# jspenmar/slowtv_monodepth

Measured on AMD Instinct MI355X. Metric: training images/sec (640×192, 3-frame) at 1/2/4/8 MI355X; warp+SSIM HBM GB/s, higher is better.
Workload: dtype f32

## Files before the change

### slowtv_monodepth_amd/conv_routing.py

```python
from __future__ import annotations

import torch

from ._lib import Unsupported

_MODE = 'auto'
_ROUTES: dict = {}
_AB_WARMUPS, _AB_ROUNDS, _AB_MARGIN = 2, 5, 0.97
_DECLINED = (Unsupported, ValueError)


def set_conv_route(mode: str = 'auto'):
    global _MODE
    if mode not in ('auto', 'mfma', 'miopen'): raise ValueError(mode)
    _MODE = mode
    _ROUTES.clear()


def conv_routes() -> dict:
    return dict(_ROUTES)


_COARSE_W_MAX, _COARSE_C_MIN = 80, 256
_Z_FWD_WGT = [dict(px_min=1000, ch_max=511), dict(px_min=2400)]
STATIC_RULES = {
    'padded': {'fwd': [dict(thin=True), dict(thin=False, px_min=20000, c_co_max=128*64), dict(thin=False, coarse=True, px_min=1000)],
               'data': [dict(thin=True), dict(thin=False, px_min=5000, c_max=256), dict(thin=False, coarse=True, px_min=1000)],
               'wgt': [dict(thin=False, px_min=20000, co_max=64), dict(thin=False, coarse=True, px_min=2400)]},
    'bf16': {'fwd': [dict(thin=True)], 'data': [dict(thin=True)], 'wgt': [dict(thin=True)]},
    'zpad': {'fwd': _Z_FWD_WGT, 'data': [dict(px_min=1000)], 'wgt': _Z_FWD_WGT},
    'stem': {'fwd': [dict(px_min=20000)], 'wgt': [dict(px_min=20000)]},
}
_FAMILY_OF_SUFFIX = {'': 'padded', 'bf16': 'bf16', 'z': 'zpad', 's': 'stem'}
_BOUNDS = {'px_min': lambda v, B, C, CO, h, w: B*h*w >= v,
           'c_max': lambda v, B, C, CO, h, w: C <= v,
           'co_max': lambda v, B, C, CO, h, w: CO <= v,
           'c_co_max': lambda v, B, C, CO, h, w: C*CO <= v,
           'ch_max': lambda v, B, C, CO, h, w: max(C, CO) <= v,
           'thin': lambda v, B, C, CO, h, w: (CO == 16) == v,
           'coarse': lambda v, B, C, CO, h, w: (w <= _COARSE_W_MAX and C >= _COARSE_C_MIN) == v}


STRIDED_RULES = {
    's2': {'fwd': [dict(px_min=5000)], 'wgt': []},
}


TRANSPOSED_RULES = {
    't2': {'data': [dict(px_min=5000)]},
}


def static_rule(op, B, C, CO, h, w) -> bool:
    kind, _, suffix = op.partition('_')
    if suffix in _FAMILY_OF_SUFFIX: clauses = STATIC_RULES[_FAMILY_OF_SUFFIX[suffix]][kind]
    elif suffix in STRIDED_RULES or suffix not in TRANSPOSED_RULES: clauses = STRIDED_RULES[suffix][kind]
    else: clauses = TRANSPOSED_RULES[suffix][kind]
    return any(all(_BOUNDS[name](v, B, C, CO, h, w) for name, v in clause.items()) for clause in clauses)


def may_serve(key, unknown=True) -> bool:
    if _MODE != 'auto': return _MODE == 'mfma'
    r = _ROUTES.get(key)
    if r is None: return static_rule(*key) if torch.cuda.is_initialized() and _capturing() else unknown
    return r[0]


_capturing = torch.cuda.is_current_stream_capturing


def _time_interleaved(run_mfma, run_ref, rounds):
    ev = [[torch.cuda.Event(enable_timing=True) for _ in range(3)] for _ in range(rounds)]
    for e in ev:
        e[0].record(); run_mfma(); e[1].record(); run_ref(); e[2].record()
    torch.cuda.synchronize()
    return [e[0].elapsed_time(e[1])*1e3 for e in ev], [e[1].elapsed_time(e[2])*1e3 for e in ev]


def _conv_route(op, B, C, CO, h, w, run_mfma, run_ref) -> bool:
    if _MODE != 'auto': return _MODE == 'mfma'
    key = (op, B, C, CO, h, w)
    r = _ROUTES.get(key)
    if r is None:
        if _capturing(): return static_rule(op, B, C, CO, h, w)
        for _ in range(_AB_WARMUPS): run_mfma(); run_ref()
        us_m, us_r = _time_interleaved(run_mfma, run_ref, _AB_ROUNDS)
        t_m, t_r = sorted(us_m)[_AB_ROUNDS//2], sorted(us_r)[_AB_ROUNDS//2]
        r = _ROUTES[key] = (t_m < _AB_MARGIN*t_r, t_m, t_r)
    return r[0]


def serve(key, run_mfma, run_ref, *, eligible, force=False):
    if not eligible: return run_ref()
    if force: return run_mfma()
    try:
        use = _conv_route(*key, run_mfma, run_ref)
    except _DECLINED:
        _ROUTES[key] = (False, float('nan'), float('nan'))
        use = False
    if use:
        try:
            return run_mfma()
        except _DECLINED:
            pass
    return run_ref()
```

### slowtv_monodepth_amd/csrc/smd_conv_s2.hip

```cpp
#include "smd_common.h"
#include "smd_kernels.h"
#include "smd_conv_mfma_dev.h"
#include <algorithm>
#include <type_traits>

namespace smd {

namespace {

constexpr int kS2Pix = 388;

template <int P>
__global__ __launch_bounds__(256, 2) void k_conv_s2_fwd(const float* __restrict__ x, const uint4* __restrict__ wp, float* __restrict__ out,
                                                        int CK, int M, int H, int W, int ho, int wo, int TR, int TCW, int KS, int kc_per_split,
                                                        size_t split_stride, unsigned gx, unsigned gy, unsigned gz) {
  constexpr int NPIX = kS2Pix, kBuf = P*NPIX*2;
  __shared__ uint4 tile[2*kBuf];
  const int lane = threadIdx.x & 63, wall = __builtin_amdgcn_readfirstlane(threadIdx.x >> 6), j = lane & 31, g = lane >> 5;
  const int MT = M >> 5, MG = (MT + 3) >> 2;
  const unsigned nblk = (unsigned)(MG*KS)*gx*gy*gz, lid = xcd_block_id(nblk);
  if (lid >= nblk) return;
  const int mg_own = (int)(lid % MG)*4 + wall, mg = min(mg_own, MT - 1), ks = (lid/MG) % KS;
  const unsigned tl = lid/(MG*KS);
  const int x0 = (int)(tl % gx)*TCW, y0 = (int)((tl/gx) % gy)*TR, b = (int)(tl/(gx*gy));
  const int PW = 2*TCW + 1, PWH = TCW + 1, NP = (2*TR + 1)*PW;
  const int KC = CK >> 4, kc0 = ks*kc_per_split, kc1 = min(KC, kc0 + kc_per_split);
  const size_t plane = (size_t)H*W;
  const float* src = x + (size_t)b*CK*plane;

  int lbase[2];
  bool have[2];
#pragma unroll
  for (int nt = 0; nt < 2; ++nt) {
    const int p = nt*32 + j, r = p/TCW, c = p - r*TCW;
    have[nt] = p < TR*TCW && y0 + r < ho && x0 + c < wo;
    lbase[nt] = have[nt] ? 2*r*PW + c : 0;
  }

  using Stage = PatchStager<256, NPIX, P, float, true>;
  constexpr int TRIPS = Stage::TRIPS;
  Stage stage;
#pragma unroll
  for (int t = 0; t < TRIPS; ++t) {
    const int item = Stage::item(t), half = item >= NPIX ? 1 : 0, pix = item - half*NPIX;
    const int rp = pix/PW, q = pix - rp*PW, col = q < PWH ? 2*q : 2*(q - PWH) + 1;
    const int yy = 2*y0 + rp - 1, xx = 2*x0 + col - 1;
    stage.pofs[t] = (pix < NP && yy >= 0 && yy < H && xx >= 0 && xx < W) ? yy*W + xx : -1;
  }
  float v[TRIPS][8];
  auto request = [&](int kc) { stage.request(src, plane, kc, v); };
  auto file_trip = [&](int buf, int t) { stage.file_trip(tile, buf, t, v); };

  f32x16 acc[2], lo[2];
#pragma unroll
  for (int nt = 0; nt < 2; ++nt)
#pragma unroll
    for (int r = 0; r < 16; ++r) { acc[nt][r] = 0.f; lo[nt][r] = 0.f; }

  bf16x8 A[5][P], Bf[2][2][P];
  const uint4* wq = wp + ((size_t)mg*KC*9*P)*64 + lane;
  auto fetch_a = [&](bf16x8 (&dst)[P], int kc, int tap) {
#pragma unroll
    for (int p = 0; p < P; ++p) dst[p] = as_frag(wq[(size_t)((kc*9 + tap)*P + p)*64]);
  };
  auto read_b = [&](bf16x8 (&dst)[2][P], int buf, int tap) {
    const int ky = tap/3, kx = tap % 3;
    const int d = ky*PW + (kx & 1)*PWH + (kx >> 1);
#pragma unroll
    for (int nt = 0; nt < 2; ++nt) Stage::read(tile, buf, lbase[nt] + d, g, dst[nt]);
  };
  auto chunk = [&](int kc, int cur, auto more_tag) {
    constexpr bool MORE = decltype(more_tag)::value;
    read_b(Bf[0], cur, 0);
#pragma unroll
    for (int tap = 0; tap < 9; ++tap) {
      if (tap < 8) read_b(Bf[(tap + 1) & 1], cur, tap + 1);
      split_mfma<P>(A[tap % 5], Bf[tap & 1], acc, lo);
      if (tap <= 4) fetch_a(A[(tap + 4) % 5], kc, tap + 4);
      else if (MORE && tap >= 6) fetch_a(A[tap - 6], kc + 1, tap - 6);
      if (MORE && tap == 8) fetch_a(A[3], kc + 1, 3);
      if (MORE && tap == 4) request(kc + 1);
      if (MORE && tap >= 6) {
#pragma unroll
        for (int t = 0; t < TRIPS; ++t) if (t*3/TRIPS == tap - 6) file_trip(cur ^ 1, t);
      }
      __builtin_amdgcn_sched_barrier(0);
    }
    __syncthreads();
  };

  if (kc0 < kc1) {
    request(kc0);
#pragma unroll
    for (int tap = 0; tap < 4; ++tap) fetch_a(A[tap], kc0, tap);
    stage.file(tile, 0, v);
  }
  __syncthreads();
  int kc = kc0;
  for (; kc + 1 < kc1; ++kc) chunk(kc, (kc - kc0) & 1, std::true_type{});
  if (kc < kc1) chunk(kc, (kc - kc0) & 1, std::false_type{});

  if (mg_own >= MT) return;
  float* dst = out + (size_t)ks*split_stride;
#pragma unroll
  for (int nt = 0; nt < 2; ++nt) {
    if (!have[nt]) continue;
    const int p = nt*32 + j, r = p/TCW, c = p - r*TCW;
#pragma unroll
    for (int rr = 0; rr < 16; ++rr) {
      const int m = mg*32 + mfma32_row(rr, g);
      dst[(((size_t)b*M + m)*ho + y0 + r)*wo + x0 + c] = acc[nt][rr] + lo[nt][rr];
    }
  }
}

__global__ __launch_bounds__(256) void k_s2_split_sum(const float* __restrict__ part, float* __restrict__ out, size_t n4, int KS) {
  const size_t i = (size_t)blockIdx.x*256 + threadIdx.x;
  if (i >= n4) return;
  const f4* p = reinterpret_cast<const f4*>(part);
  f4 s = p[i];
  for (int k = 1; k < KS; ++k) s += p[(size_t)k*n4 + i];
  reinterpret_cast<f4*>(out)[i] = s;
}

void s2_tile(int ho, int wo, int& TR, int& TCW) {
  double best = -1.0; int best_patch = 0;
  TR = 1; TCW = 1;
  for (int tcw = std::min(wo, 64); tcw >= 1; --tcw) {
    int tr = std::min(64/tcw, ho);
    while (tr > 1 && (2*tr + 1)*(2*tcw + 1) > kS2Pix) --tr;
    const int patch = (2*tr + 1)*(2*tcw + 1);
    const double useful = (double)ho*wo/((double)ceil_div(ho, tr)*ceil_div(wo, tcw)*64.0);
    if (useful > best + 1e-9 || (useful > best - 1e-9 && patch < best_patch)) { best = useful; best_patch = patch; TR = tr; TCW = tcw; }
  }
}
struct S2Shape { int TR, TCW, KS, kcs; unsigned gx, gy, gz; dim3 grid; size_t out_elems; };
S2Shape s2_fwd_shape(int B, int C, int CO, int ho, int wo) {
  S2Shape s;
  s2_tile(ho, wo, s.TR, s.TCW);
  s.gx = ceil_div(wo, s.TCW); s.gy = ceil_div(ho, s.TR); s.gz = B;
  const int KC = C >> 4, MG = ceil_div(CO >> 5, 4);
  const long long base = (long long)s.gx*s.gy*s.gz*MG;
  int ks = 1;
  if (base < 384) ks = (int)std::min<long long>(std::max(KC/2, 1), (512 + base - 1)/base);
  s.kcs = ceil_div(KC, ks); s.KS = ceil_div(KC, s.kcs);
  s.grid = dim3(8*(unsigned)ceil_div(base*s.KS, 8ll));
  s.out_elems = (size_t)B*CO*ho*wo;
  return s;
}

struct S2W {
  static constexpr int CB = 64, COB = 64, STRIP = 32, P = 3;
  static constexpr int XO = 20, XCH = 36;
  static constexpr int GCH = 20;
  static constexpr int XROW = CB*XCH, XPIECE = 3*XROW, GPIECE = COB*GCH;
  static constexpr int XITEMS = CB*2*17, XTR = (XITEMS + 255)/256;
  static constexpr int GTR = COB*8/256;
};

__global__ __launch_bounds__(256, 1) void k_conv_s2_wgrad(const float* __restrict__ x, const float* __restrict__ gy, float* __restrict__ partial,
                                                          int B, int C, int CO, int H, int W, int ho, int wo, int rows_per_block, int spb) {
  using T = S2W;
  constexpr int P = T::P, XO = T::XO, XCH = T::XCH, GCH = T::GCH, XROW = T::XROW, XPIECE = T::XPIECE, GPIECE = T::GPIECE, XTR = T::XTR, GTR = T::GTR;
  __shared__ __attribute__((aligned(16))) unsigned xs[P*XPIECE];
  __shared__ __attribute__((aligned(16))) unsigned gs[P*GPIECE];
  const int lane = threadIdx.x & 63, wv = __builtin_amdgcn_readfirstlane(threadIdx.x >> 6), j = lane & 31, g = lane >> 5;
  const int ct = wv & 1, cot = wv >> 1;
  const int CG = ceil_div(C, T::CB), COG = ceil_div(CO, T::COB);
  const int cg = blockIdx.z % CG, cog = (blockIdx.z/CG) % COG, sg = blockIdx.z/(CG*COG);
  const int x0 = blockIdx.x*T::STRIP, ybeg = blockIdx.y*rows_per_block, nrows = min(rows_per_block, ho - ybeg);
  const int b0 = sg*spb, nb = min(spb, B - b0);
  const size_t xplane = (size_t)H*W, gplane = (size_t)ho*wo;

  float xv[XTR][4], gv[GTR][4];
  auto load_x = [&](const float* xb, int ir0) {
#pragma unroll
    for (int t = 0; t < XTR; ++t) {
      const int item = t*256 + (int)threadIdx.x;
      const int d = item % 17, rr = (item/17) & 1, ch = item/34, c = cg*T::CB + ch;
      const int ir = ir0 + rr, gc = 2*x0 - 1 + 4*d;
      const bool ok = item < T::XITEMS && c < C && ir >= 0 && ir < H;
      const float* rowp = xb + ((size_t)min(c, C - 1)*H + max(min(ir, H - 1), 0))*W;
#pragma unroll
      for (int k = 0; k < 4; ++k) xv[t][k] = (ok && gc + k >= 0 && gc + k < W) ? rowp[gc + k] : 0.f;
    }
  };
  auto file_x = [&](int ir0, bool both) {
#pragma unroll
    for (int t = 0; t < XTR; ++t) {
      const int item = t*256 + (int)threadIdx.x;
      const int d = item % 17, rr = (item/17) & 1, ch = item/34;
      if (item < T::XITEMS && (both || rr == 1)) {
        const int slot = (ir0 + rr + 4) % 3;
        unsigned pe[P], po[P];
        split_pair<P>(xv[t][0], xv[t][2], pe);
        split_pair<P>(xv[t][1], xv[t][3], po);
#pragma unroll
        for (int p = 0; p < P; ++p) {
          unsigned* row = xs + p*XPIECE + slot*XROW + ch*XCH;
          row[d] = pe[p];
          if (d < 16) row[XO + d] = po[p];
        }
      }
    }
  };
  auto load_g = [&](const float* gb, int yy) {
#pragma unroll
    for (int t = 0; t < GTR; ++t) {
      const int item = t*256 + (int)threadIdx.x;
      const int chn = item >> 3, co = cog*T::COB + chn, xa = x0 + 4*(item & 7);
      const float* rowp = gb + ((size_t)min(co, CO - 1)*ho + yy)*wo;
#pragma unroll
      for (int k = 0; k < 4; ++k) gv[t][k] = (co < CO && xa + k < wo) ? rowp[xa + k] : 0.f;
    }
  };
  auto file_g = [&]() {
#pragma unroll
    for (int t = 0; t < GTR; ++t) {
      const int item = t*256 + (int)threadIdx.x;
      const int chn = item >> 3, q = item & 7;
      unsigned p0[P], p1[P];
      split_pair<P>(gv[t][0], gv[t][1], p0);
      split_pair<P>(gv[t][2], gv[t][3], p1);
#pragma unroll
      for (int p = 0; p < P; ++p) {
        gs[p*GPIECE + chn*GCH + 2*q] = p0[p];
        gs[p*GPIECE + chn*GCH + 2*q + 1] = p1[p];
      }
    }
  };

  f32x16 acc[9];
#pragma unroll
  for (int t = 0; t < 9; ++t)
#pragma unroll
    for (int r = 0; r < 16; ++r) acc[t][r] = 0.f;

  for (int s = 0; s < nb; ++s) {
    const float* xb = x + (size_t)(b0 + s)*C*xplane;
    const float* gb = gy + (size_t)(b0 + s)*CO*gplane;
    load_x(xb, 2*ybeg - 2); file_x(2*ybeg - 2, false);
    load_x(xb, 2*ybeg); file_x(2*ybeg, true);
    load_g(gb, ybeg); file_g();
    __syncthreads();
    for (int r = 0; r < nrows; ++r) {
      const int yy = ybeg + r;
      const bool more = r + 1 < nrows;
      if (more) { load_x(xb, 2*yy + 2); load_g(gb, yy + 1); }
#pragma unroll
      for (int ks = 0; ks < 2; ++ks) {
        const int kd = ks*8 + g*4;
        bf16x8 A[P];
#pragma unroll
        for (int p = 0; p < P; ++p) A[p] = as_frag(*reinterpret_cast<const uint4*>(&gs[p*GPIECE + (cot*32 + j)*GCH + kd]));
#pragma unroll
        for (int ky = 0; ky < 3; ++ky) {
          const int slot = (2*yy + ky) % 3;
          bf16x8 Bx[3][P];
#pragma unroll
          for (int p = 0; p < P; ++p) {
            const unsigned* row = xs + p*XPIECE + slot*XROW + (ct*32 + j)*XCH;
            const uint4 e = *reinterpret_cast<const uint4*>(row + kd);
            const unsigned e4 = row[kd + 4];
            Bx[0][p] = as_frag(e);
            Bx[1][p] = as_frag(*reinterpret_cast<const uint4*>(row + XO + kd));
            Bx[2][p] = as_frag(uint4{__builtin_amdgcn_alignbit(e.y, e.x, 16), __builtin_amdgcn_alignbit(e.z, e.y, 16),
                                     __builtin_amdgcn_alignbit(e.w, e.z, 16), __builtin_amdgcn_alignbit(e4, e.w, 16)});
          }
          split_mfma_sum<P>(A, Bx, &acc[ky*3]);
        }
      }
      __syncthreads();
      if (more) { file_x(2*yy + 2, true); file_g(); }
      __syncthreads();
    }
  }

  const size_t blk = ((size_t)sg*gridDim.y + blockIdx.y)*gridDim.x + blockIdx.x;
  const int c = cg*T::CB + ct*32 + j;
  if (c < C) {
#pragma unroll
    for (int t = 0; t < 9; ++t)
#pragma unroll
      for (int r = 0; r < 16; ++r) {
        const int co = cog*T::COB + cot*32 + mfma32_row(r, g);
        if (co < CO) partial[((blk*9 + t)*CO + co)*C + c] = acc[t][r];
      }
  }
}

void s2_wgrad_shape(int B, int C, int CO, int ho, int wo, dim3& grid, int& rows, int& spb) {
  const int cgs = ceil_div(C, S2W::CB)*ceil_div(CO, S2W::COB), strips = ceil_div(wo, S2W::STRIP);
  const long long base = (long long)strips*B*cgs;
  const int groups = (int)std::max(1ll, std::min<long long>(256/std::max(base, 1ll), ceil_div(ho, 6)));
  rows = ceil_div(ho, groups);
  spb = 1;
  if (rows == ho && base > 512) spb = (int)std::min<long long>(B, base/256);
  grid = dim3(strips, ceil_div(ho, rows), ceil_div(B, spb)*cgs);
}
unsigned s2_wgrad_sets(int B, int C, int CO, int ho, int wo) {
  dim3 grid; int rows, spb;
  s2_wgrad_shape(B, C, CO, ho, wo, grid, rows, spb);
  return grid.x*grid.y*(unsigned)ceil_div(B, spb);
}

constexpr int kS2DPix = 128;

__device__ __forceinline__ constexpr int s2d_slot(int s) { return (int)((0x867250134ull >> (4*s)) & 15); }

template <int P>
__device__ __forceinline__ void split_mfma_two(const bf16x8 (&A0)[P], const bf16x8 (&B0)[P], f32x16& acc0, f32x16& lo0,
                                               const bf16x8 (&A1)[P], const bf16x8 (&B1)[P], f32x16& acc1, f32x16& lo1) {
  constexpr int NPROD = n_products(P);
#pragma unroll
  for (int t = 0; t < NPROD; ++t) {
    if (t == NPROD - 1) { acc0 = mfma_bf16(A0[0], B0[0], acc0); acc1 = mfma_bf16(A1[0], B1[0], acc1); }
    else {
      lo0 = mfma_bf16(A0[prod_a(P, t)], B0[prod_b(P, t)], lo0);
      lo1 = mfma_bf16(A1[prod_a(P, t)], B1[prod_b(P, t)], lo1);
    }
  }
}

template <int P>
__global__ __launch_bounds__(256, 2) void k_conv_s2_bwd_data(const float* __restrict__ gy, const uint4* __restrict__ wp, float* __restrict__ out,
                                                             int CK, int M, int H, int W, int ho, int wo, int TR, int TCW, int KS, int kc_per_split,
                                                             size_t split_stride, unsigned gx, unsigned gyb, unsigned gz) {
  constexpr int NPIX = kS2DPix, kBuf = P*NPIX*2;
  __shared__ uint4 tile[2*kBuf];
  const int lane = threadIdx.x & 63, wall = __builtin_amdgcn_readfirstlane(threadIdx.x >> 6), j = lane & 31, g = lane >> 5;
  const int MT = (M + 31) >> 5, MG = (MT + 1) >> 1;
  const unsigned nblk = (unsigned)(MG*KS)*gx*gyb*gz, lid = xcd_block_id(nblk);
  if (lid >= nblk) return;
  const int nf = wall & 1;
  const int mt_own = (int)(lid % MG)*2 + (wall >> 1), mt = min(mt_own, MT - 1), ks = (lid/MG) % KS;
  const unsigned tl = lid/(MG*KS);
  const int c0 = (int)(tl % gx)*TCW, r0 = (int)((tl/gx) % gyb)*TR, b = (int)(tl/(gx*gyb));
  const int PW = TCW + 1, NP = (TR + 1)*PW;
  const int KC = CK >> 4, kc0 = ks*kc_per_split, kc1 = min(KC, kc0 + kc_per_split);
  const size_t plane = (size_t)ho*wo;
  const float* src = gy + (size_t)b*CK*plane;

  const int p = nf*32 + j, r = p/TCW, c = p - r*TCW;
  const bool have = p < TR*TCW && r0 + r < ho && c0 + c < wo;
  const int lbase = have ? r*PW + c : 0;

  using Stage = PatchStager<256, NPIX, P, float, true>;
  constexpr int TRIPS = Stage::TRIPS;
  Stage stage;
#pragma unroll
  for (int t = 0; t < TRIPS; ++t) {
    const int item = Stage::item(t), half = item >= NPIX ? 1 : 0, pix = item - half*NPIX;
    const int rp = pix/PW, q = pix - rp*PW;
    const int yy = r0 + rp, xx = c0 + q;
    stage.pofs[t] = (pix < NP && yy < ho && xx < wo) ? yy*wo + xx : -1;
  }
  float v[TRIPS][8];
  auto request = [&](int kc) { stage.request(src, plane, kc, v); };

  f32x16 acc[4], lo[4];
#pragma unroll
  for (int q = 0; q < 4; ++q)
#pragma unroll
    for (int rr = 0; rr < 16; ++rr) { acc[q][rr] = 0.f; lo[q][rr] = 0.f; }

  bf16x8 A[5][P], Bf[2][P];
  const uint4* wq = wp + ((size_t)mt*KC*9*P)*64 + lane;
  auto fetch_a = [&](bf16x8 (&dst)[P], int kc, int s) {
#pragma unroll
    for (int pc = 0; pc < P; ++pc) dst[pc] = as_frag(wq[(size_t)((kc*9 + s2d_slot(s))*P + pc)*64]);
  };
  auto read_b = [&](bf16x8 (&dst)[P], int buf, int d) { Stage::read(tile, buf, lbase + d, g, dst); };
  auto chunk = [&](int kc, int cur, auto more_tag) {
    constexpr bool MORE = decltype(more_tag)::value;
    read_b(Bf[0], cur, 0);
    read_b(Bf[1], cur, 1);
    split_mfma_two<P>(A[0], Bf[0], acc[0], lo[0], A[1], Bf[0], acc[1], lo[1]);
    fetch_a(A[4], kc, 4); fetch_a(A[0], kc, 5);
    __builtin_amdgcn_sched_barrier(0);
    split_mfma_two<P>(A[2], Bf[0], acc[2], lo[2], A[3], Bf[0], acc[3], lo[3]);
    fetch_a(A[1], kc, 6); fetch_a(A[2], kc, 7);
    read_b(Bf[0], cur, PW);
    if (MORE) request(kc + 1);
    __builtin_amdgcn_sched_barrier(0);
    split_mfma_two<P>(A[4], Bf[1], acc[1], lo[1], A[0], Bf[1], acc[3], lo[3]);
    fetch_a(A[3], kc, 8);
    if (MORE) fetch_a(A[0], kc + 1, 0);
    read_b(Bf[1], cur, PW + 1);
    __builtin_amdgcn_sched_barrier(0);
    split_mfma_two<P>(A[1], Bf[0], acc[2], lo[2], A[2], Bf[0], acc[3], lo[3]);
    if (MORE) { fetch_a(A[1], kc + 1, 1); fetch_a(A[2], kc + 1, 2); }
    __builtin_amdgcn_sched_barrier(0);
    split_mfma<P>(A[3], Bf[1], acc[3], lo[3]);
    if (MORE) {
      fetch_a(A[3], kc + 1, 3);
      stage.file(tile, cur ^ 1, v);
    }
    __builtin_amdgcn_sched_barrier(0);
    __syncthreads();
  };

  if (kc0 < kc1) {
    request(kc0);
#pragma unroll
    for (int s = 0; s < 4; ++s) fetch_a(A[s], kc0, s);
    stage.file(tile, 0, v);
  }
  __syncthreads();
  int kc = kc0;
  for (; kc + 1 < kc1; ++kc) chunk(kc, (kc - kc0) & 1, std::true_type{});
  if (kc < kc1) chunk(kc, (kc - kc0) & 1, std::false_type{});

  if (mt_own >= MT || !have) return;
  float* dst = out + (size_t)ks*split_stride;
  const int y = 2*(r0 + r), x = 2*(c0 + c);
  const bool row1 = y + 1 < H, col1 = x + 1 < W;
  const bool pairs = (W & 1) == 0 && (reinterpret_cast<uintptr_t>(dst) & 7) == 0;
#pragma unroll
  for (int rr = 0; rr < 16; ++rr) {
    const int m = mt*32 + mfma32_row(rr, g);
    if (m >= M) continue;
    float* q = dst + (((size_t)b*M + m)*H + y)*W + x;
    const float v00 = acc[0][rr] + lo[0][rr], v01 = acc[1][rr] + lo[1][rr], v10 = acc[2][rr] + lo[2][rr], v11 = acc[3][rr] + lo[3][rr];
    if (pairs) {
      *reinterpret_cast<f32x2v*>(q) = f32x2v{v00, v01};
      if (row1) *reinterpret_cast<f32x2v*>(q + W) = f32x2v{v10, v11};
    } else {
      q[0] = v00;
      if (col1) q[1] = v01;
      if (row1) { q[W] = v10; if (col1) q[W + 1] = v11; }
    }
  }
}

void s2d_tile(int ho, int wo, int& TR, int& TCW) {
  double best = -1.0; int best_patch = 0;
  TR = 1; TCW = 1;
  for (int tcw = std::min(wo, 63); tcw >= 1; --tcw) {
    int tr = std::min(64/tcw, ho);
    while (tr > 1 && (tr + 1)*(tcw + 1) > kS2DPix) --tr;
    const int patch = (tr + 1)*(tcw + 1);
    const double useful = (double)ho*wo/((double)ceil_div(ho, tr)*ceil_div(wo, tcw)*64.0);
    if (useful > best + 1e-9 || (useful > best - 1e-9 && patch < best_patch)) { best = useful; best_patch = patch; TR = tr; TCW = tcw; }
  }
}
S2Shape s2d_shape(int B, int C, int CO, int H, int W) {
  const int ho = (H - 1)/2 + 1, wo = (W - 1)/2 + 1;
  S2Shape s;
  s2d_tile(ho, wo, s.TR, s.TCW);
  s.gx = ceil_div(wo, s.TCW); s.gy = ceil_div(ho, s.TR); s.gz = B;
  const int KC = CO >> 4, MG = ceil_div(ceil_div(C, 32), 2);
  const long long base = (long long)s.gx*s.gy*s.gz*MG;
  int ks = 1;
  if (base < 256) ks = (int)std::min<long long>(std::max(KC/2, 1), (512 + base - 1)/base);
  s.kcs = ceil_div(KC, ks); s.KS = ceil_div(KC, s.kcs);
  s.grid = dim3(8*(unsigned)ceil_div(base*s.KS, 8ll));
  s.out_elems = (size_t)B*C*H*W;
  return s;
}

}

bool conv_s2_served(int C, int CO) { return C >= 16 && C % 16 == 0 && CO >= 32 && CO % 32 == 0; }
size_t conv_s2_workspace_floats(int B, int C, int CO, int H, int W) {
  const int ho = (H - 1)/2 + 1, wo = (W - 1)/2 + 1;
  const S2Shape s = s2_fwd_shape(B, C, CO, ho, wo);
  return std::max({(size_t)64, s.KS > 1 ? (size_t)s.KS*s.out_elems : (size_t)0, partial_sets_floats(s2_wgrad_sets(B, C, CO, ho, wo), (size_t)9*CO*C)});
}
hipError_t launch_conv_s2_fwd(const float* x, const void* wp_fwd, float* y, float* split_ws, int B, int C, int CO, int H, int W, hipStream_t st) {
  const int ho = (H - 1)/2 + 1, wo = (W - 1)/2 + 1;
  const S2Shape s = s2_fwd_shape(B, C, CO, ho, wo);
  hipLaunchKernelGGL(k_conv_s2_fwd<3>, s.grid, dim3(256), 0, st, x, (const uint4*)wp_fwd, s.KS > 1 ? split_ws : y, C, CO, H, W, ho, wo, s.TR, s.TCW, s.KS, s.kcs,
                     s.out_elems, s.gx, s.gy, s.gz);
  if (s.KS > 1) {
    const size_t n4 = s.out_elems/4;
    hipLaunchKernelGGL(k_s2_split_sum, dim3((unsigned)((n4 + 255)/256)), dim3(256), 0, st, split_ws, y, n4, s.KS);
  }
  return hipGetLastError();
}
hipError_t launch_conv_s2_bwd_wgt(const float* x, const float* gy, float* g_w, float* partial, int B, int C, int CO, int H, int W, hipStream_t st) {
  const int ho = (H - 1)/2 + 1, wo = (W - 1)/2 + 1;
  dim3 grid; int rows, spb;
  s2_wgrad_shape(B, C, CO, ho, wo, grid, rows, spb);
  hipLaunchKernelGGL(k_conv_s2_wgrad, grid, dim3(256), 0, st, x, gy, partial, B, C, CO, H, W, ho, wo, rows, spb);
  return launch_partial_sets_finalize(partial, grid.x*grid.y*(unsigned)ceil_div(B, spb), 9*CO*C, SetIndexMap{CO, C}, g_w, st);
}

long long conv_s2d_blocks(int B, int C, int CO, int H, int W) { return (long long)s2d_shape(B, C, CO, H, W).grid.x; }
size_t conv_s2d_workspace_floats(int B, int C, int CO, int H, int W) {
  const S2Shape s = s2d_shape(B, C, CO, H, W);
  return std::max((size_t)64, s.KS > 1 ? (size_t)s.KS*s.out_elems : (size_t)0);
}
hipError_t launch_conv_s2_bwd_data(const float* gy, const void* wp_bwd, float* g_x, float* split_ws, int B, int C, int CO, int H, int W, hipStream_t st) {
  const int ho = (H - 1)/2 + 1, wo = (W - 1)/2 + 1;
  const S2Shape s = s2d_shape(B, C, CO, H, W);
  hipLaunchKernelGGL(k_conv_s2_bwd_data<3>, s.grid, dim3(256), 0, st, gy, (const uint4*)wp_bwd, s.KS > 1 ? split_ws : g_x, CO, C, H, W, ho, wo, s.TR, s.TCW, s.KS,
                     s.kcs, s.out_elems, s.gx, s.gy, s.gz);
  if (s.KS > 1) {
    const size_t n4 = s.out_elems/4;
    hipLaunchKernelGGL(k_s2_split_sum, dim3((unsigned)((n4 + 255)/256)), dim3(256), 0, st, split_ws, g_x, n4, s.KS);
  }
  return hipGetLastError();
}

}
```

Measured before the change: 959.3.

## Rewrite stride-2 conv weight-grad kernel with async LDS DMA ring and enable routing

Replaces the register-staged load/split/store pipeline of the stride-2 weight-gradient kernel with direct buffer-to-LDS DMA into a four-slot ring. Loads are issued ahead and waited on with vmcnt. The bf16 split now happens at fragment-build time, and each input row is reused across two output rows via alternating accumulator sets. Tile shape changes to 32 input by 128 output channels on a 16-wide strip with two blocks per CU. The grid shape is now picked by a small cost model. The static routing rule is also enabled for small-C shapes during graph capture. The aim is to hide global-load latency and cut register pressure, at the cost of tricky wait-count logic and reduced channel reuse per block.

```diff
diff --git a/slowtv_monodepth_amd/conv_routing.py b/slowtv_monodepth_amd/conv_routing.py
--- a/slowtv_monodepth_amd/conv_routing.py
+++ b/slowtv_monodepth_amd/conv_routing.py
@@ -42,7 +42,7 @@
 
 
 STRIDED_RULES = {
-    's2': {'fwd': [dict(px_min=5000)], 'wgt': []},
+    's2': {'fwd': [dict(px_min=5000)], 'wgt': [dict(c_max=64, px_min=5000)]},
 }
 
 
diff --git a/slowtv_monodepth_amd/csrc/smd_conv_s2.hip b/slowtv_monodepth_amd/csrc/smd_conv_s2.hip
--- a/slowtv_monodepth_amd/csrc/smd_conv_s2.hip
+++ b/slowtv_monodepth_amd/csrc/smd_conv_s2.hip
@@ -150,84 +150,60 @@
 }
 
 struct S2W {
-  static constexpr int CB = 64, COB = 64, STRIP = 32, P = 3;
-  static constexpr int XO = 20, XCH = 36;
-  static constexpr int GCH = 20;
-  static constexpr int XROW = CB*XCH, XPIECE = 3*XROW, GPIECE = COB*GCH;
-  static constexpr int XITEMS = CB*2*17, XTR = (XITEMS + 255)/256;
-  static constexpr int GTR = COB*8/256;
+  static constexpr int CB = 32, COB = 128, STRIP = 16, P = 3, NW = 4, D = 4;
+  static constexpr int XCS = 36, GCS = 20, XDW = CB*XCS, GDW = COB*GCS, SLOT = 2*XDW + GDW;
+  static constexpr int NX = 16*XCS/64, NG = 16*GCS/64, NDMA = NX + 2*NG;
+  static_assert(NX*64 == 16*XCS && NG*64 == 16*GCS && 2*XDW == NW*NX*64 && GDW == NW*2*NG*64, "a wave: sixteen channels of one input row, 32 of dL/dy");
+  static_assert((D - 2)*NDMA < 64 && D == 4, "the waits below are immediates of six bits, for a ring of four");
 };
 
-__global__ __launch_bounds__(256, 1) void k_conv_s2_wgrad(const float* __restrict__ x, const float* __restrict__ gy, float* __restrict__ partial,
+__global__ __launch_bounds__(256, 2) void k_conv_s2_wgrad(const float* __restrict__ x, const float* __restrict__ gy, float* __restrict__ partial,
                                                           int B, int C, int CO, int H, int W, int ho, int wo, int rows_per_block, int spb) {
   using T = S2W;
-  constexpr int P = T::P, XO = T::XO, XCH = T::XCH, GCH = T::GCH, XROW = T::XROW, XPIECE = T::XPIECE, GPIECE = T::GPIECE, XTR = T::XTR, GTR = T::GTR;
-  __shared__ __attribute__((aligned(16))) unsigned xs[P*XPIECE];
-  __shared__ __attribute__((aligned(16))) unsigned gs[P*GPIECE];
+  constexpr int P = T::P, D = T::D, XCS = T::XCS, GCS = T::GCS, XDW = T::XDW, SLOT = T::SLOT, NX = T::NX, NG = T::NG, NDMA = T::NDMA;
+  __shared__ __attribute__((aligned(16))) unsigned lds[D*SLOT];
   const int lane = threadIdx.x & 63, wv = __builtin_amdgcn_readfirstlane(threadIdx.x >> 6), j = lane & 31, g = lane >> 5;
-  const int ct = wv & 1, cot = wv >> 1;
+  const int cot = wv;
   const int CG = ceil_div(C, T::CB), COG = ceil_div(CO, T::COB);
   const int cg = blockIdx.z % CG, cog = (blockIdx.z/CG) % COG, sg = blockIdx.z/(CG*COG);
   const int x0 = blockIdx.x*T::STRIP, ybeg = blockIdx.y*rows_per_block, nrows = min(rows_per_block, ho - ybeg);
-  const int b0 = sg*spb, nb = min(spb, B - b0);
+  const int b0 = sg*spb, nsteps = nrows + 1, nsteps_all = min(spb, B - b0)*nsteps;
   const size_t xplane = (size_t)H*W, gplane = (size_t)ho*wo;
-
-  float xv[XTR][4], gv[GTR][4];
-  auto load_x = [&](const float* xb, int ir0) {
-#pragma unroll
-    for (int t = 0; t < XTR; ++t) {
-      const int item = t*256 + (int)threadIdx.x;
-      const int d = item % 17, rr = (item/17) & 1, ch = item/34, c = cg*T::CB + ch;
-      const int ir = ir0 + rr, gc = 2*x0 - 1 + 4*d;
-      const bool ok = item < T::XITEMS && c < C && ir >= 0 && ir < H;
-      const float* rowp = xb + ((size_t)min(c, C - 1)*H + max(min(ir, H - 1), 0))*W;
-#pragma unroll
-      for (int k = 0; k < 4; ++k) xv[t][k] = (ok && gc + k >= 0 && gc + k < W) ? rowp[gc + k] : 0.f;
-    }
-  };
-  auto file_x = [&](int ir0, bool both) {
-#pragma unroll
-    for (int t = 0; t < XTR; ++t) {
-      const int item = t*256 + (int)threadIdx.x;
-      const int d = item % 17, rr = (item/17) & 1, ch = item/34;
-      if (item < T::XITEMS && (both || rr == 1)) {
-        const int slot = (ir0 + rr + 4) % 3;
-        unsigned pe[P], po[P];
-        split_pair<P>(xv[t][0], xv[t][2], pe);
-        split_pair<P>(xv[t][1], xv[t][3], po);
-#pragma unroll
-        for (int p = 0; p < P; ++p) {
-          unsigned* row = xs + p*XPIECE + slot*XROW + ch*XCH;
-          row[d] = pe[p];
-          if (d < 16) row[XO + d] = po[p];
-        }
-      }
-    }
-  };
-  auto load_g = [&](const float* gb, int yy) {
-#pragma unroll
-    for (int t = 0; t < GTR; ++t) {
-      const int item = t*256 + (int)threadIdx.x;
-      const int chn = item >> 3, co = cog*T::COB + chn, xa = x0 + 4*(item & 7);
-      const float* rowp = gb + ((size_t)min(co, CO - 1)*ho + yy)*wo;
-#pragma unroll
-      for (int k = 0; k < 4; ++k) gv[t][k] = (co < CO && xa + k < wo) ? rowp[xa + k] : 0.f;
-    }
-  };
-  auto file_g = [&]() {
-#pragma unroll
-    for (int t = 0; t < GTR; ++t) {
-      const int item = t*256 + (int)threadIdx.x;
-      const int chn = item >> 3, q = item & 7;
-      unsigned p0[P], p1[P];
-      split_pair<P>(gv[t][0], gv[t][1], p0);
-      split_pair<P>(gv[t][2], gv[t][3], p1);
-#pragma unroll
-      for (int p = 0; p < P; ++p) {
-        gs[p*GPIECE + chn*GCH + 2*q] = p0[p];
-        gs[p*GPIECE + chn*GCH + 2*q + 1] = p1[p];
-      }
-    }
+  const unsigned lds0 = (unsigned)__builtin_amdgcn_readfirstlane((int)(unsigned)(unsigned long long)(__attribute__((address_space(3))) unsigned*)lds);
+
+  const int xrow = wv >> 1, xc0 = cg*T::CB + (wv & 1)*16, gc0 = cog*T::COB + wv*32;
+  const bool x_live = xc0 < C, g_live = gc0 < CO;
+  unsigned vx[NX], vg[NG];
+#pragma unroll
+  for (int n = 0; n < NX; ++n) {
+    const int d = n*64 + lane, ch = d/XCS, col = d - ch*XCS, ix = 2*x0 - 1 + col;
+    vx[n] = (col <= 2*T::STRIP && ix >= 0 && ix < W) ? (unsigned)(ch*(H*W) + ix)*4u : 0x80000000u;
+  }
+#pragma unroll
+  for (int n = 0; n < NG; ++n) {
+    const int d = n*64 + lane, ch = d/GCS, col = d - ch*GCS;
+    vg[n] = (col < T::STRIP && x0 + col < wo) ? (unsigned)(ch*(ho*wo) + x0 + col)*4u : 0x80000000u;
+  }
+  const rsrc_t rs_0 = make_rsrc(x, 0);
+
+  int is_b = b0, is_r = 0;
+  auto issue = [&](int q) {
+    const int y = ybeg + is_r, b = is_b;
+    const bool last = is_r == nrows;
+    if (++is_r == nsteps) { is_r = 0; ++is_b; }
+    const unsigned base = lds0 + (unsigned)((q % D)*SLOT*4);
+    const int yx = 2*y - 1 + xrow;
+    const bool x_in = x_live && yx >= 0 && yx < H && !(last && xrow == 1), g_in = g_live && !last;
+    const rsrc_t rx = x_in ? make_rsrc(x + ((size_t)b*C + xc0)*xplane, 16*xplane*4) : rs_0;
+    const rsrc_t rg0 = g_in ? make_rsrc(gy + ((size_t)b*CO + gc0)*gplane, 16*gplane*4) : rs_0;
+    const rsrc_t rg1 = g_in ? make_rsrc(gy + ((size_t)b*CO + gc0 + 16)*gplane, 16*gplane*4) : rs_0;
+    const unsigned sx = x_in ? (unsigned)yx*(unsigned)W*4u : 0u, sgo = g_in ? (unsigned)y*(unsigned)wo*4u : 0u;
+#pragma unroll
+    for (int n = 0; n < NX; ++n) lds_dma_dword(rx, vx[n], sx, base + (unsigned)((wv*NX + n)*256));
+#pragma unroll
+    for (int n = 0; n < NG; ++n) lds_dma_dword(rg0, vg[n], sgo, base + (unsigned)(2*XDW*4 + (wv*2*NG + n)*256));
+#pragma unroll
+    for (int n = 0; n < NG; ++n) lds_dma_dword(rg1, vg[n], sgo, base + (unsigned)(2*XDW*4 + (wv*2*NG + NG + n)*256));
   };
 
   f32x16 acc[9];
@@ -235,49 +211,69 @@
   for (int t = 0; t < 9; ++t)
 #pragma unroll
     for (int r = 0; r < 16; ++r) acc[t][r] = 0.f;
-
-  for (int s = 0; s < nb; ++s) {
-    const float* xb = x + (size_t)(b0 + s)*C*xplane;
-    const float* gb = gy + (size_t)(b0 + s)*CO*gplane;
-    load_x(xb, 2*ybeg - 2); file_x(2*ybeg - 2, false);
-    load_x(xb, 2*ybeg); file_x(2*ybeg, true);
-    load_g(gb, ybeg); file_g();
-    __syncthreads();
-    for (int r = 0; r < nrows; ++r) {
-      const int yy = ybeg + r;
-      const bool more = r + 1 < nrows;
-      if (more) { load_x(xb, 2*yy + 2); load_g(gb, yy + 1); }
-#pragma unroll
-      for (int ks = 0; ks < 2; ++ks) {
-        const int kd = ks*8 + g*4;
-        bf16x8 A[P];
-#pragma unroll
-        for (int p = 0; p < P; ++p) A[p] = as_frag(*reinterpret_cast<const uint4*>(&gs[p*GPIECE + (cot*32 + j)*GCH + kd]));
-#pragma unroll
-        for (int ky = 0; ky < 3; ++ky) {
-          const int slot = (2*yy + ky) % 3;
-          bf16x8 Bx[3][P];
-#pragma unroll
-          for (int p = 0; p < P; ++p) {
-            const unsigned* row = xs + p*XPIECE + slot*XROW + (ct*32 + j)*XCH;
-            const uint4 e = *reinterpret_cast<const uint4*>(row + kd);
-            const unsigned e4 = row[kd + 4];
-            Bx[0][p] = as_frag(e);
-            Bx[1][p] = as_frag(*reinterpret_cast<const uint4*>(row + XO + kd));
-            Bx[2][p] = as_frag(uint4{__builtin_amdgcn_alignbit(e.y, e.x, 16), __builtin_amdgcn_alignbit(e.z, e.y, 16),
-                                     __builtin_amdgcn_alignbit(e.w, e.z, 16), __builtin_amdgcn_alignbit(e4, e.w, 16)});
-          }
-          split_mfma_sum<P>(A, Bx, &acc[ky*3]);
-        }
-      }
-      __syncthreads();
-      if (more) { file_x(2*yy + 2, true); file_g(); }
-      __syncthreads();
-    }
+  bf16x8 A[2][P];
+#pragma unroll
+  for (int r = 0; r < 2; ++r)
+#pragma unroll
+    for (int p = 0; p < P; ++p) A[r][p] = as_frag(uint4{0u, 0u, 0u, 0u});
+
+  auto x_frags = [&](const float* row, bf16x8 (&Bx)[3][P]) {
+    const f4 q0 = *reinterpret_cast<const f4*>(row), q1 = *reinterpret_cast<const f4*>(row + 4), q2 = *reinterpret_cast<const f4*>(row + 8),
+             q3 = *reinterpret_cast<const f4*>(row + 12);
+    const float q4 = row[16];
+    unsigned pe[5][P], po[4][P];
+    split_pair<P>(q0.x, q0.z, pe[0]); split_pair<P>(q1.x, q1.z, pe[1]); split_pair<P>(q2.x, q2.z, pe[2]); split_pair<P>(q3.x, q3.z, pe[3]); split_pair<P>(q4, 0.f, pe[4]);
+    split_pair<P>(q0.y, q0.w, po[0]); split_pair<P>(q1.y, q1.w, po[1]); split_pair<P>(q2.y, q2.w, po[2]); split_pair<P>(q3.y, q3.w, po[3]);
+#pragma unroll
+    for (int p = 0; p < P; ++p) {
+      Bx[0][p] = as_frag(uint4{pe[0][p], pe[1][p], pe[2][p], pe[3][p]});
+      Bx[1][p] = as_frag(uint4{po[0][p], po[1][p], po[2][p], po[3][p]});
+      Bx[2][p] = as_frag(uint4{__builtin_amdgcn_alignbit(pe[1][p], pe[0][p], 16), __builtin_amdgcn_alignbit(pe[2][p], pe[1][p], 16),
+                               __builtin_amdgcn_alignbit(pe[3][p], pe[2][p], 16), __builtin_amdgcn_alignbit(pe[4][p], pe[3][p], 16)});
+    }
+  };
+
+  int st_r = 0;
+  auto step = [&](int i, bf16x8 (&a0)[P], const bf16x8 (&a1)[P]) {
+    const int il = st_r;
+    if (++st_r == nsteps) st_r = 0;
+    const int after = min(D - 2, nsteps_all - 1 - i);
+    if (after >= 2) asm volatile("s_waitcnt vmcnt(%0)" :: "n"(2*NDMA) : "memory");
+    else if (after == 1) asm volatile("s_waitcnt vmcnt(%0)" :: "n"(NDMA) : "memory");
+    else asm volatile("s_waitcnt vmcnt(0)" ::: "memory");
+    __builtin_amdgcn_s_barrier();
+    asm volatile("" ::: "memory");
+    if (i + D - 1 < nsteps_all) issue(i + D - 1);
+    const float* slot = reinterpret_cast<const float*>(lds) + (i % D)*SLOT;
+    const float* xo = slot + j*XCS + g*16;
+    bf16x8 Bx[3][P];
+    const bool own = il < nrows;
+    if (own) {
+      const float* gr = slot + 2*XDW + (cot*32 + j)*GCS + g*8;
+      const f4 g0 = *reinterpret_cast<const f4*>(gr), g1 = *reinterpret_cast<const f4*>(gr + 4);
+      unsigned pg[4][P];
+      split_pair<P>(g0.x, g0.y, pg[0]); split_pair<P>(g0.z, g0.w, pg[1]); split_pair<P>(g1.x, g1.y, pg[2]); split_pair<P>(g1.z, g1.w, pg[3]);
+#pragma unroll
+      for (int p = 0; p < P; ++p) a0[p] = as_frag(uint4{pg[0][p], pg[1][p], pg[2][p], pg[3][p]});
+    }
+    x_frags(xo, Bx);
+    if (own) split_mfma_sum<P>(a0, Bx, &acc[0]);
+    if (il > 0) split_mfma_sum<P>(a1, Bx, &acc[6]);
+    if (own) {
+      x_frags(xo + XDW, Bx);
+      split_mfma_sum<P>(a0, Bx, &acc[3]);
+    }
+  };
+  issue(0);
+  issue(1);
+  if (nsteps_all > 2) issue(2);
+  for (int i = 0; i < nsteps_all; i += 2) {
+    step(i, A[0], A[1]);
+    if (i + 1 < nsteps_all) step(i + 1, A[1], A[0]);
   }
 
   const size_t blk = ((size_t)sg*gridDim.y + blockIdx.y)*gridDim.x + blockIdx.x;
-  const int c = cg*T::CB + ct*32 + j;
+  const int c = cg*T::CB + j;
   if (c < C) {
 #pragma unroll
     for (int t = 0; t < 9; ++t)
@@ -290,13 +286,25 @@
 }
 
 void s2_wgrad_shape(int B, int C, int CO, int ho, int wo, dim3& grid, int& rows, int& spb) {
-  const int cgs = ceil_div(C, S2W::CB)*ceil_div(CO, S2W::COB), strips = ceil_div(wo, S2W::STRIP);
-  const long long base = (long long)strips*B*cgs;
-  const int groups = (int)std::max(1ll, std::min<long long>(256/std::max(base, 1ll), ceil_div(ho, 6)));
-  rows = ceil_div(ho, groups);
-  spb = 1;
-  if (rows == ho && base > 512) spb = (int)std::min<long long>(B, base/256);
-  grid = dim3(strips, ceil_div(ho, rows), ceil_div(B, spb)*cgs);
+  const long long per = (long long)ceil_div(C, S2W::CB)*ceil_div(CO, S2W::COB)*ceil_div(wo, S2W::STRIP);
+  const double set_us = 2.0*9.0*CO*C*4.0/6e6;
+  auto cost = [&](long long blocks, int steps, long long sets) {
+    return 1.8*steps*(double)ceil_div(blocks, 256ll)*(blocks > 256 ? 0.65 : 1.0) + set_us*(double)sets;
+  };
+  const long long strips = ceil_div(wo, S2W::STRIP);
+  double best = -1.0;
+  rows = ho; spb = 1;
+  for (int groups = 1; groups <= std::max(1, ho/4); ++groups) {
+    const int r = ceil_div(ho, groups), bands = ceil_div(ho, r);
+    const double t = cost(per*B*bands, r + 1, strips*bands*B);
+    if (best < 0 || t < best) { best = t; rows = r; }
+  }
+  for (int s = 2; s <= B; ++s) {
+    const int nsg = ceil_div(B, s);
+    const double t = cost(per*nsg, s*(ho + 1), strips*nsg);
+    if (t < best) { best = t; rows = ho; spb = s; }
+  }
+  grid = dim3(ceil_div(wo, S2W::STRIP), ceil_div(ho, rows), (unsigned)(ceil_div(B, spb)*(per/ceil_div(wo, S2W::STRIP))));
 }
 unsigned s2_wgrad_sets(int B, int C, int CO, int ho, int wo) {
   dim3 grid; int rows, spb;
```

After: 960.7 (median of 2 runs). About the same (+0.2%).
